# Farama-Foundation/Miniworld

Hardware: AMD Instinct MI355X
Metric: env-steps/s (batched, 80x60 RGB) (higher is better)
Workload: dtype f32

## Files before the change

include/mwengine.h:

```cpp
#ifndef MWENGINE_H
#define MWENGINE_H
#include <stdint.h>
#ifdef __cplusplus
extern "C" {
#endif

#define MW_ABI_VERSION 4

enum {
    MW_OK = 0,
    MW_E_INVALID = -1,
    MW_E_HIP = -2,
    MW_E_NOMEM = -3,
    MW_E_CAPACITY = -4,
    MW_E_DEVICE = -5,
    MW_E_OVERFLOW = -6
};

enum { MW_ENT_NONE = 0, MW_ENT_BOX = 1, MW_ENT_MESH = 2, MW_ENT_FRAME = 3 };

enum {
    MW_TASK_NONE = 0,
    MW_TASK_GOTO = 1,
    MW_TASK_PICKUP = 2,
// ... 246 lines not shown
int mw_debug_set_nav_passes(mw_engine *e, int32_t *d_passes);

int mw_check(mw_engine *e, void *stream);

int mw_kernel_time_ms(mw_engine *e, int32_t reset, double *raster_ms, double *setup_ms, int64_t *launches);

int mw_get_info(mw_engine *e, int32_t *d_health, double *d_ent_pos, int32_t ent_slot, void *stream);
int mw_get_final_info(mw_engine *e, int32_t *d_health, double *d_goal_pos, void *stream);
int mw_get_reset_pending(mw_engine *e, uint8_t *d_out, void *stream);

int mw_set_frame_reuse(mw_engine *e, int32_t on);
int mw_get_frame_clean(mw_engine *e, uint8_t *d_out, void *stream);

int mw_set_frame_cache(mw_engine *e, int32_t slots);
int mw_get_frame_source(mw_engine *e, uint8_t *d_out, void *stream);

int mw_get_list_lengths(mw_engine *e, int32_t first_env, int32_t count, int32_t *host_out, void *stream);

int mw_debug_set_mesh_frame_seq(mw_engine *e, uint32_t seq);
int mw_debug_get_slow_heads(mw_engine *e, uint32_t *host_out, void *stream);

enum { MW_PATH_TILE = 0, MW_PATH_QUAD = 1, MW_PATH_QUAD_MESH = 2, MW_PATH_GENERIC = 3 };
int mw_raster_path(const mw_engine *e);

#ifdef __cplusplus
}
#endif
#endif
```

miniworld_amd/csrc/mw_engine.h:

```cpp
#pragma once
#include <hip/hip_runtime.h>

#include <algorithm>
#include <cstdarg>
#include <cstdio>
#include <cstdlib>
#include <memory>
#include <string>
#include <utility>
#include <vector>

#include "mw_assets.h"
#include "mw_device.h"
#include "mw_kernels.h"
#include "mw_policy.h"

#define MW_TIMING_STRIDE 8

template <typename H, hipError_t (*destroy)(H)>
struct Destroy { void operator()(H h) const { (void)destroy(h); } };
template <typename T>
using DevBuf = std::unique_ptr<T, Destroy<void *, hipFree>>;
using Stream = std::unique_ptr<ihipStream_t, Destroy<hipStream_t, hipStreamDestroy>>;
using Event = std::unique_ptr<ihipEvent_t, Destroy<hipEvent_t, hipEventDestroy>>;
// ... 79 lines not shown
    bool frame_reuse = false;
    struct { uint8_t *obs = nullptr; float *depth = nullptr; int layout = 0; bool valid = false; } held;
    struct {
        int slots = 0;
        DevBuf<uint8_t> frames;
        DevBuf<float> depth;
        DevBuf<uint64_t> meta;
        DevBuf<MwFcArgs> d_args;
        MwFcArgs args{};
        bool args_stale = true;
        bool with_depth = false;
        bool dirty = true;
    } fc;
    uint32_t *d_plan[2] = {nullptr, nullptr};
    int plan_cur = 0;
    struct {
        int depth = 0, pad = 0, layout = 0, cur = 0;
        uint8_t *ring = nullptr, *final_stack = nullptr;
        size_t frame_bytes = 0;
        int64_t pushes = 0;
        uint8_t *flags = nullptr;
    } stack;
    MwSnapConfig snap_cfg{};
    MwSnapLayout snap_layout{};
    MwSnapTable *d_snap_tab = nullptr;
    int snap_chunks_per_item = 0;
    Event ev_refill_done;
};

namespace mwhost {
// ... 124 lines not shown
```

miniworld_amd/csrc/mw_engine.hip:

```cpp
#include <cmath>
#include <cstring>

#include "mw_engine.h"
#include "mw_rng.h"

namespace mwhost {
thread_local std::string g_create_error;
}
using namespace mwhost;

namespace {

void seed_env(const mw_engine *e, uint64_t *rng, int i, uint64_t seed)
{
    const size_t N = (size_t)e->cfg.num_envs;
    uint64_t w[5];
    mw::rng_seed_words(e->cfg.rng_mode == MW_RNG_PCG64, seed, w);
    for (int k = 0; k < 5; ++k) rng[(size_t)k * N + i] = w[k];
}

int upload_textures(mw_engine *e)
{
    const size_t table = (size_t)MW_MAX_TEX * sizeof(MwTexDesc) / 4;
    size_t total = table;
// ... 159 lines not shown
    ALLOC(a.rec_cull, (size_t)N * a.max_vis * MW_CULL_REC);
    if (has_visiting_order(cfg->max_visible)) {
        ALLOC(a.rec_order, (size_t)N * (a.max_vis + 1));
    }
    if (cfg->max_polys > 64 && !(getenv("MW_OCC_CACHE") && atoi(getenv("MW_OCC_CACHE")) == 0)) {
        ALLOC(a.occ_valid, e->n_sets);
        ALLOC(a.occ_cache, (size_t)e->n_sets * MW_OCC_CACHE_STRIDE(cfg->max_polys));
    }
    { const auto pick = [](int id) { return id >= MW_SC_pending_remove; }; MW_WORLD_FIELDS(LIVE_ALLOC) }
    ALLOC(a.frame_clean, (size_t)N);
    ALLOC(a.fc_key, (size_t)MW_FC_KEY_WORDS * N); ALLOC(a.fc_epoch, (size_t)N); ALLOC(a.fc_source, (size_t)N);
    HIP_TRY(e, hipMemset(a.pending_remove, 0xFF, 4 * (size_t)N));
    ALLOC(a.nvis, N); ALLOC(a.envhdr, (size_t)MW_ENVHDR * N); ALLOC(a.status, 1);
    ALLOC(e->d_reward_scratch, N); ALLOC(e->d_flag_scratch, 2 * (size_t)N);
    ALLOC(e->d_final_list, 1 + (size_t)N);
    ALLOC(e->d_plan[0], MW_PLAN_WORDS(N)); ALLOC(e->d_plan[1], MW_PLAN_WORDS(N));
    ALLOC(e->stack.flags, 2 * (size_t)N);
    ALLOC(e->d_mask, N); ALLOC(e->d_step_override, 3 * (size_t)N);
#ifdef MW_PERF_HOOKS
    if (getenv("MW_K1_PROF")) ALLOC(a.k1_prof, MW_K1_PROF_SLOTS * (size_t)N);
    if (getenv("MW_ENT_PROF")) ALLOC(e->d_ent_prof, (size_t)16 * 2 * N * MW_MAX_MESH_ENTS * 8);
    if (getenv("MW_K2Q_PROF")) ALLOC(e->d_k2q_prof, (size_t)N * 96);
#endif
#undef LIVE_ALLOC
#undef ALLOC
    {
        std::vector<int32_t> m1((size_t)N, -1);
        HIP_TRY(e, hipMemcpy(a.carry, m1.data(), 4 * (size_t)N, hipMemcpyHostToDevice));
        std::vector<uint64_t> seeds(5 * (size_t)N, 0);
        for (int i = 0; i < N; ++i) seed_env(e, seeds.data(), i, (uint64_t)i);
        HIP_TRY(e, hipMemcpy(a.rng, seeds.data(), 40 * (size_t)N, hipMemcpyHostToDevice));
// ... 516 lines not shown
    if (!d_health && !d_goal_pos) return fail(e, MW_E_INVALID, "mw_get_final_info: nothing asked for");
    if (d_health && !e->args.final_health) return fail(e, MW_E_INVALID, "mw_get_final_info: this engine's task keeps no health (MW_TASK_COLLECT only)");
    return launch_info(e, 1, e->args.final_health, e->args.final_goal, 0, d_health, d_goal_pos, stream);
}

int mw_get_reset_pending(mw_engine *e, uint8_t *d_out, void *stream)
{
    return e ? get_env_bytes(e, "mw_get_reset_pending", e->args.reset_pending, d_out, stream) : MW_E_INVALID;
}

int mw_get_frame_source(mw_engine *e, uint8_t *d_out, void *stream)
{
    return e ? get_env_bytes(e, "mw_get_frame_source", e->args.fc_source, d_out, stream) : MW_E_INVALID;
}

int mw_get_frame_clean(mw_engine *e, uint8_t *d_out, void *stream)
{
    return e ? get_env_bytes(e, "mw_get_frame_clean", e->args.frame_clean, d_out, stream) : MW_E_INVALID;
}

int mw_kernel_time_ms(mw_engine *e, int32_t reset, double *raster_ms, double *setup_ms, int64_t *launches)
{
    if (!e) return MW_E_INVALID;
    ON_DEVICE(e);
    double r = 0, s = 0;
    int64_t n = 0;
    for (auto &ev : e->ev_used) {
        (void)hipEventSynchronize(ev.c.get());
        float t1 = 0, t2 = 0;
        (void)hipEventElapsedTime(&t1, ev.a.get(), ev.b.get());
// ... 20 lines not shown
```

miniworld_amd/csrc/mw_engine_frame.hip:

```cpp
#include "mw_engine.h"

using namespace mwhost;

namespace {

template <typename K>
K k1_of(const mw_engine *e, int lanes, K wave, K wave_pcg, K dense, K dense_pcg)
{
    const bool pcg = e->cfg.rng_mode == MW_RNG_PCG64;
    if (lanes) return pcg ? dense_pcg : dense;
    return pcg ? wave_pcg : wave;
}
#define MW_K1(e, lanes, stem) k1_of(e, lanes, stem##_kernel, stem##_pcg_kernel, stem##_dense_kernel, stem##_dense_pcg_kernel)

template <typename... A>
struct KernelPair {
    void (*plain)(A...);
    void (*sub)(A..., const int32_t *);
};
template <typename... A>
KernelPair<A...> kernel_pair(void (*plain)(A...), void (*sub)(A..., const int32_t *)) { return {plain, sub}; }
#define MW_PAIR(stem) kernel_pair(stem##_kernel, stem##_sub_kernel)

template <typename... A, typename... P>
// ... 205 lines not shown
void launch_quad(const mw_engine *e, const Frame &f, int part, hipStream_t st, const uint32_t *plan = nullptr)
{
    const MwArgs &a = f.a;
    const int lds = mw_rasterq_lds_bytes(e->cfg.msaa, a.W, a.H, a.n_tiles, f.depth ? 1 : 0);
    launch(f.p.quad4 ? MW_PAIR(mw_rasterq4) : MW_PAIR(mw_rasterq), f.list, dim3(e->cfg.num_envs), dim3(MWQ_THREADS), (size_t)lds, st, a.N, a.W, a.H, a.max_vis,
           a.tiles_x, a.n_tiles, (const float *)a.rec_raster, (const float *)a.rec_shade, (const float *)a.rec_cull,
           (const int32_t *)a.nvis, (const float *)a.envhdr, a.texels, f.obs, f.depth, raster_flags(e->dbg_flags, e->obs_layout, part, 0u, false), e->texel_bytes, e->d_k2q_prof,
           plan && f.pol.cache ? (const MwFcArgs *)e->fc.d_args.get() : nullptr, plan);
}

const uint32_t *launch_plan(mw_engine *e, const Frame &f, hipStream_t st)
{
    const MwArgs &a = f.a; const int N = e->cfg.num_envs;
    uint32_t *plan = e->d_plan[e->plan_cur], *next = e->d_plan[e->plan_cur ^ 1];
    e->plan_cur ^= 1;
    hipLaunchKernelGGL(mw_frame_plan_kernel, dim3((N + MW_PLAN_ENVS - 1) / MW_PLAN_ENVS), dim3(64), 0, st, N, f.pol.reuse ? 1 : 0, (const uint8_t *)a.frame_clean,
                       (const uint64_t *)a.fc_key, f.pol.cache ? (const uint64_t *)e->fc.meta.get() : nullptr, f.pol.cache ? e->fc.slots : 0, a.fc_source, plan, next);
    return plan;
}

void launch_tiles(const mw_engine *e, const Frame &f, int part, hipStream_t st)
{
    const MwArgs &a = f.a; const mw_engine::MeshPath &m = e->mp;
    const TileLaunch t = tile_launch(part, a.tile_list != nullptr, f.p.big, a.max_vis, a.n_tiles, e->waves_per_env, e->cfg.num_envs, m.mesh_tile_waves);
    launch(tile_kernel_of(f.p.big, f.p.depth, f.p.general, f.p.ragged, f.p.mesh, t.part == 1), f.list, dim3(t.grid), dim3(64), t.lds, st,
           a.N, a.W, a.H, a.max_vis, a.tiles_x, a.n_tiles, t.waves_per_env, t.tiles_per_wave, (const float *)a.rec_raster, (const float *)a.rec_shade,
           (const float *)a.rec_cull, (const int32_t *)a.nvis, (const float *)a.envhdr, a.tex, a.texels, f.obs, f.depth, raster_flags(e->dbg_flags, e->obs_layout, t.part, f.mf.stamp, f.pol.reuse),
           e->texel_bytes, (const uint16_t *)a.rec_order, a.mesh_pos, a.mesh_nrm, a.mesh_rgb, a.mesh_uv, m.keys.get(),
           (const float *)m.plane_cache.get(), m.plane_cap, (const float4 *)m.slow_frags.get(), (const uint32_t *)m.slow_head.get(),
           (const uint32_t *)a.tile_list, a.ent_list_n, a.tile_list_cap, std::max(a.n_xcc, 1), (const uint8_t *)a.frame_clean);
}

// ... 366 lines not shown
```

miniworld_amd/csrc/mw_engine_kernels.hip:

```cpp
#include "mw_kernels.h"

extern "C" __global__ void mw_info_kernel(int N, int E, const int32_t *health, const double *epos, int slot, int32_t *out_health, double *out_pos)
{
    const int i = blockIdx.x * blockDim.x + threadIdx.x;
    if (i >= N) return;
    if (out_health) out_health[i] = health[i];
    if (out_pos)
        for (int c = 0; c < 3; ++c) out_pos[(size_t)i * 3 + c] = epos[((size_t)c * E + slot) * N + i];
}

extern "C" __global__ __launch_bounds__(1024) void mw_final_list_kernel(int N, const uint8_t *__restrict__ pending, int32_t *__restrict__ pending_remove,
                                                                       int32_t *__restrict__ list)
{
    __shared__ int s_wave[16];
    const int tid = (int)threadIdx.x, lane = tid & 63, wave = tid >> 6;
    int base = 0;
    for (int i0 = 0; i0 < N; i0 += 1024) {
        const int i = i0 + tid;
        const bool p = i < N && pending[i] != 0;
        const unsigned long long m = __ballot(p);
        if (lane == 0) s_wave[wave] = __popcll(m);
        __syncthreads();
        int before = base, total = 0;
        for (int w = 0; w < 16; ++w) {
// ... 18 lines not shown
    if ((int)blockIdx.x >= list[0]) return;
    const size_t env = (size_t)list[1 + blockIdx.x];
    const uint8_t *src = obs + env * row_bytes;
    uint8_t *dst = final_obs + env * row_bytes;
    if ((((uintptr_t)obs | (uintptr_t)final_obs | (uintptr_t)row_bytes) & 15u) == 0) {
        for (size_t k = threadIdx.x; k < row_bytes / 16; k += blockDim.x)
            reinterpret_cast<uint4 *>(dst)[k] = reinterpret_cast<const uint4 *>(src)[k];
    } else {
        for (size_t k = threadIdx.x; k < row_bytes; k += blockDim.x) dst[k] = src[k];
    }
    if (depth && final_depth)
        for (int k = threadIdx.x; k < depth_row; k += blockDim.x) final_depth[env * depth_row + k] = depth[env * depth_row + k];
}

extern "C" __global__ __launch_bounds__(64) void mw_frame_plan_kernel(int N, int reuse, const uint8_t *__restrict__ frame_clean, const uint64_t *__restrict__ key,
                                                                     const uint64_t *__restrict__ meta, int slots, uint8_t *__restrict__ frame_source,
                                                                     uint32_t *__restrict__ plan, uint32_t *__restrict__ next)
{
    const int lane = (int)threadIdx.x, env = (int)blockIdx.x * MW_PLAN_ENVS + lane;
    if (blockIdx.x == 0 && lane < 2) next[lane] = 0u;
    const bool on = env < N;
    uint32_t v = MW_SRC_CLEAN;
    if (on) {
        const bool clean = frame_clean[env] != 0;
        uint32_t match = 0u, header = 0u;
        if (meta) {
            const uint64_t *row = static_cast<const uint64_t *>(__builtin_assume_aligned(meta + (size_t)env * MW_FC_META_WORDS(slots), 16));
            const uint64_t *cur = static_cast<const uint64_t *>(__builtin_assume_aligned(key + (size_t)env * MW_FC_KEY_WORDS, 16));
            header = (uint32_t)row[0];
#pragma unroll
            for (int j = 0; j < MW_FC_MAX_SLOTS; ++j) {
                const int jj = j < slots ? j : slots - 1;
                match |= mw_fc_key_equal(static_cast<const uint64_t *>(__builtin_assume_aligned(row + 2 + MW_FC_KEY_WORDS * jj, 16)), cur) && j < slots ? 1u << j : 0u;
            }
        }
        v = mw_frame_verdict(clean, reuse != 0, match, header, meta ? slots : 0);
        frame_source[env] = (uint8_t)v;
    }
    const uint32_t src = v & 0xFFu;
    const bool draw = on && src == MW_SRC_DRAWN, copy = on && src >= (uint32_t)MW_SRC_SLOT(0);
    const uint64_t md = __builtin_amdgcn_ballot_w64(draw), mc = __builtin_amdgcn_ballot_w64(copy), below = (1ull << lane) - 1ull;
    unsigned long long base = 0ull;
    if (lane == 0 && (md | mc))
        base = atomicAdd(reinterpret_cast<unsigned long long *>(plan), (unsigned long long)__popcll(md) | (unsigned long long)__popcll(mc) << 32);
    const uint32_t bd = (uint32_t)__builtin_amdgcn_readfirstlane((int)(uint32_t)base), bc = (uint32_t)__builtin_amdgcn_readfirstlane((int)(uint32_t)(base >> 32));
    const uint32_t entry = (uint32_t)env | (v >> 8) << MW_PLAN_ENV_BITS;
    const uint32_t id = bd + (uint32_t)__popcll(md & below), ic = bc + (uint32_t)__popcll(mc & below);
    if (draw && id < (uint32_t)N) plan[MW_PLAN_HEAD + id] = entry;
    if (copy && ic < (uint32_t)N) plan[MW_PLAN_HEAD + (size_t)N + ic] = entry;
}
```

miniworld_amd/csrc/mw_frame_plan.h:

```cpp
#pragma once
#include <stdint.h>

#include "mw_hd.h"

#ifndef MW_FC_KEY_WORDS
#define MW_FC_KEY_WORDS 10
#define MW_FC_META_WORDS(slots) (2 + MW_FC_KEY_WORDS * (slots))
#define MW_FC_MAX_SLOTS 8
#endif

#define MW_SRC_DRAWN 0
#define MW_SRC_CLEAN 1
#define MW_SRC_SLOT(j) (2 + (j))

#define MW_PLAN_HEAD 4
#define MW_PLAN_WORDS(N) (MW_PLAN_HEAD + 2 * (size_t)(N))
#define MW_PLAN_ENV_BITS 24
#define MW_PLAN_ENV_MASK 0xFFFFFFu

MW_HD uint32_t mw_frame_verdict(bool clean, bool reuse, uint32_t match, uint32_t header, int slots)
{
    if (reuse && clean) return MW_SRC_CLEAN;
    if (slots <= 0) return MW_SRC_DRAWN;
    match &= (1u << slots) - 1u;
    if (match) {
        uint32_t hit = 0;
        while (!((match >> hit) & 1u)) ++hit;
        return (uint32_t)MW_SRC_SLOT(hit) | hit << 8;
    }
    const uint32_t last = (uint32_t)(slots - 1);
    return MW_SRC_DRAWN | (header < last ? header : last) << 8;
}

// ... 15 lines not shown
```

miniworld_amd/csrc/mw_kernels.h:

```cpp
#pragma once
#include "mw_device.h"
#include "mw_frame_plan.h"
#include "mw_snapshot.h"
#include "mw_snapframes.h"
#include "mw_state_view.h"
#include "mw_nav.h"

#define MW_KERNEL_PAIR(stem, ...)                          \
    extern "C" __global__ void stem##_kernel(__VA_ARGS__); \
    extern "C" __global__ void stem##_sub_kernel(__VA_ARGS__, const int32_t *list)

#define MW_K1_ARGS MwArgs a, int lanes_per_env, const int32_t *__restrict__ actions, float *__restrict__ reward, \
                   uint8_t *__restrict__ term, uint8_t *__restrict__ trunc
extern "C" __global__ void mw_step_setup_kernel(MW_K1_ARGS);
extern "C" __global__ void mw_step_setup_pcg_kernel(MW_K1_ARGS);
extern "C" __global__ void mw_step_setup_dense_kernel(MW_K1_ARGS);
extern "C" __global__ void mw_step_setup_dense_pcg_kernel(MW_K1_ARGS);
#define MW_K1_REPEAT_ARGS MW_K1_ARGS, int repeat, int32_t *__restrict__ nsteps
extern "C" __global__ void mw_step_repeat_kernel(MW_K1_REPEAT_ARGS);
extern "C" __global__ void mw_step_repeat_pcg_kernel(MW_K1_REPEAT_ARGS);
extern "C" __global__ void mw_step_repeat_dense_kernel(MW_K1_REPEAT_ARGS);
extern "C" __global__ void mw_step_repeat_dense_pcg_kernel(MW_K1_REPEAT_ARGS);
#define MW_K1_PLAN_ARGS MW_K1_ARGS, int horizon, int32_t *__restrict__ nsteps, float *__restrict__ step_reward, int frameless
extern "C" __global__ void mw_step_plan_kernel(MW_K1_PLAN_ARGS);
// ... 108 lines not shown

#define MW_SNAPF_ARGS MwSnapfArgs a, uint32_t *__restrict__ status
extern "C" __global__ void mw_snapshot_save_frames_kernel(MW_SNAPF_ARGS, const uint8_t *__restrict__ obs, const uint8_t *__restrict__ depth,
                                                          const uint8_t *__restrict__ ring, const uint8_t *__restrict__ stack_flags,
                                                          uint8_t *__restrict__ frames, MW_SNAP_ITEMS);
extern "C" __global__ void mw_snapshot_load_frames_kernel(MW_SNAPF_ARGS, const uint8_t *__restrict__ frames, uint8_t *__restrict__ obs,
                                                          uint8_t *__restrict__ depth, uint8_t *__restrict__ ring, uint8_t *__restrict__ stack_flags,
                                                          MW_SNAP_ITEMS);

extern "C" __global__ void mw_info_kernel(int N, int E, const int32_t *health, const double *epos, int slot, int32_t *out_health, double *out_pos);
extern "C" __global__ void mw_final_list_kernel(int N, const uint8_t *__restrict__ pending, int32_t *__restrict__ pending_remove, int32_t *__restrict__ list);
extern "C" __global__ void mw_final_copy_kernel(const int32_t *__restrict__ list, const uint8_t *__restrict__ obs, uint8_t *__restrict__ final_obs,
                                                unsigned long long row_bytes, const float *__restrict__ depth, float *__restrict__ final_depth, int depth_row);
#define MW_PLAN_ENVS 64
extern "C" __global__ void mw_frame_plan_kernel(int N, int reuse, const uint8_t *__restrict__ frame_clean, const uint64_t *__restrict__ key,
                                                const uint64_t *__restrict__ meta, int slots, uint8_t *__restrict__ frame_source,
                                                uint32_t *__restrict__ plan, uint32_t *__restrict__ next);

#define MW_SV_THREADS 256
#define MW_SV_ENVS (MW_SV_THREADS / 64)
extern "C" __global__ void mw_state_get_kernel(MwStateArrays a, mw_state_view v, int N, int E, int first_env, int count);
extern "C" __global__ void mw_state_set_where_kernel(MwStateArrays a, mw_state_view v, const uint8_t *__restrict__ mask, int N, int E,
                                                     uint32_t *__restrict__ status, uint8_t *__restrict__ reset_pending,
                                                     uint8_t *__restrict__ frame_clean, uint32_t *__restrict__ fc_epoch,
                                                     uint8_t *__restrict__ stack_flags);

#define MW_NAV_THREADS 512
#define MW_NAV_QUERY_THREADS 256
extern "C" __global__ void mw_nav_build_kernel(MwNavArgs a, mw_nav_params p, const uint8_t *__restrict__ mask, const double *__restrict__ d_target,
                                               uint16_t *__restrict__ field, int32_t *__restrict__ passes);
extern "C" __global__ void mw_nav_query_kernel(MwNavArgs a, mw_nav_params p, const double *__restrict__ d_target, const uint16_t *__restrict__ field,
                                               const double *__restrict__ pos, int32_t *__restrict__ cost, int32_t *__restrict__ next,
// ... 5 lines not shown
```

miniworld_amd/csrc/mw_policy.h:

```cpp
#pragma once
#include <stddef.h>
#include <stdint.h>

#include "../../include/mwengine.h"
#include "mw_shape.h"
#include "mw_snapframes.h"
#include "mw_snapshot.h"

namespace mwpolicy {

inline bool tile_kernels_exact(int W, int H) { return W <= 128 && H <= 128 && W * H <= 128 * 96; }

inline int tiles_across(int W) { return (W + MW_TILE_W - 1) / MW_TILE_W; }
inline int tiles_down(int H) { return (H + MW_TILE_H - 1) / MW_TILE_H; }
inline bool frame_on_grid(int W, int H) { return W % MW_TILE_W == 0 && H % MW_TILE_H == 0; }
inline bool tile_path_ok(int W, int H) { return frame_on_grid(W, H) && tile_kernels_exact(W, H); }
inline bool frame_size_ok(int W, int H) { return W >= 1 && H >= 1 && W <= 255 * MW_TILE_W && H <= 255 * MW_TILE_H; }

inline bool has_visiting_order(int max_visible) { return max_visible > 64; }

inline int geom_lanes(int max_polys, int max_ents, bool order)
{
    const int items = 2 * (max_polys + 6 * max_ents + 1);
    int L = 8;
// ... 101 lines not shown
};
inline FramePolicy frame_policy(const FrameFacts &f)
{
    const bool plain = (f.kind == CALL_RENDER || f.kind == CALL_STEP) && f.view_flags == 0;
    const bool seeded_pass = f.seeded && (f.kind == CALL_TERMINAL_STEP || f.kind == CALL_LIST_PASS) && f.view_flags == 0;
    const bool plain_step = (plain && f.kind == CALL_STEP) || (seeded_pass && f.kind == CALL_TERMINAL_STEP), bare = !f.meshes && f.dbg_flags == 0;
    const bool source = plain_step && f.path == MW_PATH_QUAD;
    return {f.frame_reuse && plain_step && bare && f.held_match, source,
            source && f.cache_allocated && bare && f.layout == MW_OBS_HWC_U8 && f.task != MW_TASK_COLLECT, plain || seeded_pass};
}

inline bool frame_plans(const FramePolicy &pol, int path, bool listed, int N)
{
    return !listed && path == MW_PATH_QUAD && (pol.reuse || pol.cache) && N <= 0xFFFFFF;
}

struct TileLaunch { int part, waves_per_env, tiles_per_wave, grid; size_t lds; };
inline TileLaunch tile_launch(int part, bool tile_list, bool big, int max_vis, int n_tiles, int wpe, int N, int mesh_tile_waves)
{
    const int lds_recs = max_vis < MW_LDS_RECS ? max_vis : MW_LDS_RECS;
    const size_t lds = big ? 192 : (size_t)lds_recs * (MW_LDS_SHADE_Q + MW_LDS_CULL_Q) * 16 + 192;
    const bool listed = part == 2 && tile_list;
    if (listed) part = 3;
    const int wpe2 = part == 2 ? n_tiles : wpe, tpw2 = part == 2 ? 1 : (n_tiles + wpe - 1) / wpe;
    const int all = N * n_tiles;
    return {part, wpe2, tpw2, listed ? (mesh_tile_waves < all ? mesh_tile_waves : all) : (N + 7) / 8 * 8 * wpe2, lds};
}

inline bool wide_units(uintptr_t bits) { return (bits & 15u) == 0; }

// ... 41 lines not shown
```

miniworld_amd/csrc/mw_rasterq.hip:

```cpp
#include "mw_mesh.h"
#include "mw_kernels.h"

#define MWQ_WAVES (MWQ_THREADS / 64)
#define MWQ_CAP_MAX 48
#define MWQ_SLOTS 16
#define MWQ_EMPTY 63u
#ifndef MWQ_TILE_FALLBACK
#define MWQ_TILE_FALLBACK 1
#endif
#ifndef MWQ_OCC
#define MWQ_OCC 6
#endif

namespace {

__device__ inline bool wave_all(bool p) { return __builtin_amdgcn_ballot_w64(p) == __builtin_amdgcn_read_exec(); }
__device__ inline bool wave_any(bool p) { return __builtin_amdgcn_ballot_w64(p) != 0ull; }

enum { QC_FALLBACK = 0, QC_BIG, QC_EXACT, QC_P4, QC_P3, QC_P2, QC_P1, QC_TRIV, QC_SKY, QC_NCLS, QC_NONE = 15 };

template <int S> struct QRec {
    static constexpr int TQ = (S + 3) / 4;
    static constexpr int SH = 4 + 3 * TQ;
    static constexpr int CT = SH + 6;
// ... 439 lines not shown
        wins &= valid;
        if (!wave_any(wins)) continue;
        const float4 *rec = recp(valid ? p : 0);
        const RGB c = shade_lane(rec + QRec<S>::SH, cx.te, fx + 0.5f, fy + 0.5f);
#pragma unroll
        for (int s = 0; s < S; ++s) {
            const bool eq = valid && pid[s] == (uint32_t)p;
            q.r[s] = eq ? c.r : q.r[s]; q.g[s] = eq ? c.g : q.g[s]; q.b[s] = eq ? c.b : q.b[s];
        }
    }
    store_pixel<S>(cx, q, key[0] >> 16, px, py, on);
}

#ifdef MW_PERF_HOOKS
#define MWQ_WG_BEGIN() const unsigned long long wg_t0 = prof ? __builtin_amdgcn_s_memrealtime() : 0ull
#define MWQ_WG_END(kind) do { if (prof && (threadIdx.x & 63) == 0) { unsigned long long *w_ = prof + (size_t)N * (MWQ_WAVES * 8 + 16) + (size_t)blockIdx.x * 16; \
    if (threadIdx.x == 0) { w_[0] = wg_t0; w_[1] = (kind); } w_[2 + (threadIdx.x >> 6)] = __builtin_amdgcn_s_memrealtime(); } } while (0)
#else
#define MWQ_WG_BEGIN() do {} while (0)
#define MWQ_WG_END(kind) do {} while (0)
#endif
template <int S, bool SUB = false>
__device__ inline void rasterq_body(
    int N, int W, int H, int max_vis, int tiles_x, int n_tiles,
    const float *__restrict__ rec_raster, const float *__restrict__ rec_shade, const float *__restrict__ rec_cull,
    const int32_t *__restrict__ nvis_arr, const float *__restrict__ envhdr, const uint32_t *__restrict__ texels,
    uint8_t *__restrict__ obs, float *__restrict__ depth, int dbg, int texel_bytes, unsigned long long *__restrict__ prof,
    const MwFcArgs *__restrict__ fc, const uint32_t *__restrict__ plan, const int32_t *__restrict__ list = nullptr)
{
    extern __shared__ __attribute__((aligned(16))) unsigned char smem[];
    typedef QRec<S> R;
    MWQ_WG_BEGIN();
    int env = blockIdx.x;
    const int tid = threadIdx.x, lane = tid & 63, wave = tid >> 6;
    const bool has_depth = depth != nullptr;
    uint32_t fc_victim = 0u;
    if (SUB) {
        if (env >= list[0]) return;
        env = list[1 + env];
    } else if (env >= N) return;
    else if (plan) {
        const uint32_t b = blockIdx.x, n_draw = plan[0];
        if (b < n_draw) {
            const uint32_t entry = plan[MW_PLAN_HEAD + b];
            env = (int)(entry & MW_PLAN_ENV_MASK);
            fc_victim = entry >> MW_PLAN_ENV_BITS;
        } else {
            if (b - n_draw >= plan[1] || !fc) { MWQ_WG_END(3); return; }
            const uint32_t entry = plan[MW_PLAN_HEAD + (size_t)N + (b - n_draw)];
            env = (int)(entry & MW_PLAN_ENV_MASK);
            const int hit = (int)(entry >> MW_PLAN_ENV_BITS), fc_slots = fc->slots;
            const int fbytes = W * H * 3;
            const uint8_t *src = fc->frames + ((size_t)env * fc_slots + hit) * fbytes;
            uint8_t *dst = obs + (size_t)env * fbytes;
            if ((reinterpret_cast<uintptr_t>(dst) & 15u) == 0u)
                for (int i = tid; i < fbytes / 16; i += MWQ_THREADS) reinterpret_cast<uint4 *>(dst)[i] = reinterpret_cast<const uint4 *>(src)[i];
            else if ((reinterpret_cast<uintptr_t>(dst) & 3u) == 0u)
                for (int i = tid; i < fbytes / 4; i += MWQ_THREADS) reinterpret_cast<uint32_t *>(dst)[i] = reinterpret_cast<const uint32_t *>(src)[i];
            else
                for (int i = tid; i < fbytes; i += MWQ_THREADS) dst[i] = src[i];
            if (has_depth) {
                const float *zs = fc->depth + ((size_t)env * fc_slots + hit) * (W * H);
                float *zd = depth + (size_t)env * (W * H);
                if ((reinterpret_cast<uintptr_t>(zd) & 15u) == 0u)
                    for (int i = tid; i < W * H / 4; i += MWQ_THREADS) reinterpret_cast<float4 *>(zd)[i] = reinterpret_cast<const float4 *>(zs)[i];
                else
                    for (int i = tid; i < W * H; i += MWQ_THREADS) zd[i] = zs[i];
            }
            MWQ_WG_END(2);
            return;
        }
    }
    const QPlan pl = q_plan(S, W, H, n_tiles, has_depth);
    float4 *s_rec = reinterpret_cast<float4 *>(smem + pl.rec);
    uint8_t *s_frame = smem + pl.frame;
    uint16_t *s_z = reinterpret_cast<uint16_t *>(smem + pl.zbuf);
    uint32_t *s_qids = reinterpret_cast<uint32_t *>(smem + pl.qids);
    uint16_t *s_queue = reinterpret_cast<uint16_t *>(smem + pl.queue);
    uint16_t *s_xq = reinterpret_cast<uint16_t *>(smem + pl.xq);
    uint32_t *s_tcnt = reinterpret_cast<uint32_t *>(smem + pl.tcnt);
    uint32_t *s_tfull = reinterpret_cast<uint32_t *>(smem + pl.tfull);
    uint8_t *s_tlist = smem + pl.tlist;
    uint32_t *s_tmask = reinterpret_cast<uint32_t *>(smem + pl.tmask);
    uint32_t *s_pe = reinterpret_cast<uint32_t *>(smem + pl.pe);
// ... 231 lines not shown
            const int Q = Q0 + tid;
            const uint32_t cls = Q < nquads ? s_qids[Q] >> 24 : (uint32_t)QC_NONE;
            const uint32_t base = (uint32_t)__builtin_amdgcn_ds_bpermute((int)(cls & 15u) << 2, (int)fb_lane);
            if (cls != QC_NONE) s_queue[base * 16u + s_rank[Q]] = (uint16_t)Q;
        }
        for (uint32_t b = tid; b < first_bat[QC_NCLS]; b += MWQ_THREADS) {
            uint32_t cls = 0u;
#pragma unroll
            for (int c = 1; c < QC_NCLS; ++c) cls += b >= first_bat[c] ? 1u : 0u;
            uint32_t cfirst = 0u, cslot = 0u, ccnt = 0u;
#pragma unroll
            for (int c = 0; c < QC_NCLS; ++c) { cfirst = cls == (uint32_t)c ? first_bat[c] : cfirst; cslot = cls == (uint32_t)c ? first_b[c] : cslot; ccnt = cls == (uint32_t)c ? cnt_c[c] : ccnt; }
            const uint32_t size = cls == QC_TRIV ? 64u : 16u, bi = b - cfirst;
            s_btab[b] = ((cslot + bi * (size / 16u)) * 16u) | (cls << 12) | (min(size, ccnt - bi * size) << 16);
        }
        __syncthreads();

        stamp(4);
        if (prof && tid < QC_NCLS) prof[(size_t)N * MWQ_WAVES * 8 + (size_t)env * 16 + tid] = s_misc[tid];
        const uint32_t sky_u8 = sky_bytes<S>(cx);
        const uint32_t n_batches = (dbg & 0x400) ? 0u : first_bat[QC_NCLS];
        for (;;) {
            uint32_t b = 0u;
            if (lane == 0) b = atomicAdd(&s_misc[17], 1u);
            b = (uint32_t)__builtin_amdgcn_readfirstlane((int)b);
            if (b >= n_batches) break;
            const uint32_t be = (uint32_t)__builtin_amdgcn_readfirstlane((int)s_btab[b]);
            const int cls = (int)((be >> 12) & 15u);
            if ((dbg & 0x800) && cls != QC_TRIV) continue;
            if ((dbg & 0x1000) && cls == QC_TRIV) continue;
// ... 110 lines not shown
    if (!SUB && fc) {
        const int fc_slots = fc->slots;
        const uint32_t victim = s_misc[20];
        uint64_t *meta = fc->meta + (size_t)env * MW_FC_META_WORDS(fc_slots);
        uint4 *fd = reinterpret_cast<uint4 *>(fc->frames + ((size_t)env * fc_slots + victim) * (npix * 3));
        const uint4 *src = reinterpret_cast<const uint4 *>(s_frame);
        for (int i = tid; i < npix * 3 / 16; i += MWQ_THREADS) fd[i] = src[i];
        if (has_depth) {
            float *fz = fc->depth + ((size_t)env * fc_slots + victim) * npix;
            for (int i = tid; i < npix; i += MWQ_THREADS) fz[i] = depth_of(i);
        }
        if (tid < MW_FC_KEY_WORDS / 2)
            reinterpret_cast<uint4 *>(meta + 2 + MW_FC_KEY_WORDS * victim)[tid] = reinterpret_cast<const uint4 *>(fc->key + (size_t)env * MW_FC_KEY_WORDS)[tid];
        if (tid == 64) meta[0] = (uint64_t)(victim + 1u == (uint32_t)fc_slots ? 0u : victim + 1u);
    }
    MWQ_WG_END(0);
}

}

#define MWQ_FWD N, W, H, max_vis, tiles_x, n_tiles, rec_raster, rec_shade, rec_cull, nvis_arr, envhdr, texels, obs, depth, dbg, texel_bytes, prof, fc, plan
#define MWQ_PAIR(stem, bounds, ...)                                                                          \
    extern "C" __global__ bounds void stem##_kernel(MWQ_ARGS) { rasterq_body<__VA_ARGS__, false>(MWQ_FWD); } \
    extern "C" __global__ bounds void stem##_sub_kernel(MWQ_ARGS, const int32_t *__restrict__ list) { rasterq_body<__VA_ARGS__, true>(MWQ_FWD, list); }
MWQ_PAIR(mw_rasterq, __launch_bounds__(MWQ_THREADS, MWQ_OCC), 8)
MWQ_PAIR(mw_rasterq4, __launch_bounds__(MWQ_THREADS), 4)

extern "C" int mw_rasterq_lds_bytes(int S, int W, int H, int n_tiles, int depth) { return q_plan(S, W, H, n_tiles, depth != 0).total; }
extern "C" int mw_rasterq_cap(int depth) { return q_cap(depth != 0); }

#ifdef MWQ_PROBE
// ... 16 lines not shown
```

miniworld_amd/engine.py:

```python
from __future__ import annotations

import ctypes as C
import os
import subprocess

import numpy as np

_CSRC = os.path.join(os.path.dirname(os.path.abspath(__file__)), "csrc")
LIB_PATH = os.environ.get("MW_ENGINE_LIB") or os.path.join(_CSRC, "libmwengine.so")

ABI_VERSION = 4
MAX_REPEAT = 256
MAX_PLAN = MAX_REPEAT
MAX_STACK = 16
STACK_PAD_RESET, STACK_PAD_ZERO = 0, 1
SNAPF_DEPTH, SNAPF_STACK = 1, 2
ENT_NONE, ENT_BOX, ENT_MESH, ENT_FRAME = 0, 1, 2, 3
POLY_ENTITY = 0x100
POLY_XF = 0x200
POLY_QUAD = 0x400
TASK_NONE, TASK_GOTO, TASK_PICKUP, TASK_PUTNEXT, TASK_SIDEWALK, TASK_SIGN, TASK_COLLECT = 0, 1, 2, 3, 4, 5, 6
GEN_NONE, GEN_HALLWAY, GEN_ONEROOM, GEN_PICKUP, GEN_MAZE, GEN_PROGRAM = 0, 1, 2, 3, 4, 5
OP_COIN, OP_DRAW_DIR, OP_PLACE, OP_FIXED, OP_BOX_SIZE, OP_COLOR, OP_APPEND = 1, 2, 3, 4, 5, 6, 7
PROG_MAX_ROOMS, PROG_MAX_TEX, PROG_MAX_OPS, PROG_MAX_ENTS = 16, 8, 48, 64
AUTORESET_OFF, AUTORESET_SAME_STEP, AUTORESET_NEXT_STEP = 0, 1, 2
OBS_HWC_U8, OBS_CWH_U8, OBS_GREY_F64 = 0, 1, 2
RNG_PHILOX, RNG_PCG64 = 0, 1
PATH_TILE, PATH_QUAD, PATH_QUAD_MESH, PATH_GENERIC = 0, 1, 2, 3

EXPORTS = [
    "mw_create", "mw_destroy", "mw_last_error", "mw_upload_texture", "mw_upload_mesh",
    "mw_set_geometry", "mw_get_geometry", "mw_set_state", "mw_get_state", "mw_set_step_params", "mw_reset",
    "mw_step", "mw_step_repeat", "mw_step_plan", "mw_step_plan_trace", "mw_render", "mw_render_top", "mw_render_view", "mw_visible_ents", "mw_set_obs_layout", "mw_pcg64_draws", "mw_check", "mw_kernel_time_ms", "mw_raster_path", "mw_get_info", "mw_get_final_info", "mw_get_reset_pending", "mw_set_frame_reuse", "mw_get_frame_clean", "mw_set_frame_cache", "mw_get_frame_source", "mw_set_final_obs", "mw_get_list_lengths", "mw_debug_set_mesh_frame_seq", "mw_debug_get_slow_heads",
    "mw_set_gen_program", "mw_selftest_rcp", "mw_selftest_div", "mw_selftest_sort", "mw_selftest_q",
    "mw_selftest_sincosf",
    "mw_set_frame_stack", "mw_stack_refresh", "mw_stack_window",
    "mw_snapshot_bytes", "mw_snapshot_save", "mw_snapshot_load",
    "mw_snapshot_frames_bytes", "mw_snapshot_save_frames", "mw_snapshot_load_frames",
    "mw_snapshot_save_at", "mw_snapshot_save_frames_at", "mw_snapshot_load_where", "mw_snapshot_load_frames_where",
    "mw_reset_where", "mw_set_reset_seeds",
    "mw_get_state_device", "mw_set_state_where",
    "mw_nav_build", "mw_nav_query", "mw_debug_set_nav_passes",
]


class MwRange(C.Structure):
    _fields_ = [("default", C.c_double), ("lo", C.c_double), ("hi", C.c_double)]

# ... 179 lines not shown
    L.mw_snapshot_save_at.argtypes = [vp, vp, vp, i32, vp, i32, vp]
    L.mw_snapshot_save_frames_at.argtypes = [vp, vp, vp, i32, vp, vp, vp, i32, i32, vp]
    L.mw_snapshot_load_where.argtypes = [vp, vp, vp, vp, i32, i32, vp]
    L.mw_snapshot_load_frames_where.argtypes = [vp, vp, vp, vp, i32, i32, i32, vp, vp, vp]
    L.mw_pcg64_draws.argtypes = [C.c_uint64, i32, vp, vp]
    L.mw_check.argtypes = [vp, vp]
    L.mw_kernel_time_ms.argtypes = [vp, i32, C.POINTER(C.c_double), C.POINTER(C.c_double), C.POINTER(C.c_int64)]
    L.mw_raster_path.argtypes = [vp]
    L.mw_get_info.argtypes = [vp, vp, vp, i32, vp]
    L.mw_get_final_info.argtypes = [vp, vp, vp, vp]
    L.mw_get_reset_pending.argtypes = [vp, vp, vp]
    L.mw_set_frame_reuse.argtypes = [vp, i32]
    L.mw_get_frame_clean.argtypes = [vp, vp, vp]
    L.mw_set_frame_cache.argtypes = [vp, i32]
    L.mw_get_frame_source.argtypes = [vp, vp, vp]
    L.mw_get_list_lengths.argtypes = [vp, i32, i32, vp, vp]
    L.mw_debug_set_mesh_frame_seq.argtypes = [vp, C.c_uint32]
    L.mw_debug_get_slow_heads.argtypes = [vp, vp, vp]
    _lib = L
    return L


def frame_reuse_allowed() -> bool:
    return os.environ.get("MW_FRAME_REUSE", "1").strip() != "0"


MAX_FRAME_CACHE = 8


def frame_cache_allowed() -> bool:
# ... 515 lines not shown
    def set_frame_reuse(self, on: bool):
        on = bool(on) and frame_reuse_allowed()
        self._check(self.lib.mw_set_frame_reuse(self.h, int(on)), "mw_set_frame_reuse")
        self.frame_reuse = on
        return on

    def set_frame_cache(self, slots: int):
        slots = int(slots) if frame_cache_allowed() else 0
        self._check(self.lib.mw_set_frame_cache(self.h, slots), "mw_set_frame_cache")
        self.frame_cache = slots
        return slots

    def get_frame_source(self, out=None):
        return self._get_bytes("mw_get_frame_source", out)

    def get_frame_clean(self, out=None):
        return self._get_bytes("mw_get_frame_clean", out)

    def list_lengths(self):
        out = np.zeros(self.N, np.int32)
        self._check(self.lib.mw_get_list_lengths(self.h, 0, self.N, out.ctypes.data, _stream_ptr(self.device)), "mw_get_list_lengths")
        return out

    def raster_path(self):
        return int(self.lib.mw_raster_path(self.h))

    def kernel_time_ms(self, reset=0):
        r, s, n = C.c_double(), C.c_double(), C.c_int64()
        self._check(self.lib.mw_kernel_time_ms(self.h, reset, C.byref(r), C.byref(s), C.byref(n)), "mw_kernel_time_ms")
        return r.value, s.value, n.value
# ... 31 lines not shown
```

Measured before the change: 17.04 million.

## Order drawn frames by visible-list cost class so heavy envs launch first

The frame plan kernel now buckets drawn environments into eight cost classes by their visible-primitive count and counts them with per-class packed atomics. The quad raster kernel maps block indices to classes from heaviest to lightest, so expensive environments start first and the tail imbalance shrinks. It costs extra ballots and atomics in the plan kernel, a larger plan buffer, and some index arithmetic per raster block. A host-side plan readback API and extra profiling fields are added as well.

```diff
diff --git a/include/mwengine.h b/include/mwengine.h
--- a/include/mwengine.h
+++ b/include/mwengine.h
@@ -284,6 +284,7 @@
 
 int mw_set_frame_cache(mw_engine *e, int32_t slots);
 int mw_get_frame_source(mw_engine *e, uint8_t *d_out, void *stream);
+int mw_get_frame_plan(mw_engine *e, uint32_t *host_plan, int64_t words, int32_t *host_lengths, void *stream);
 
 int mw_get_list_lengths(mw_engine *e, int32_t first_env, int32_t count, int32_t *host_out, void *stream);
 
diff --git a/miniworld_amd/csrc/mw_engine.h b/miniworld_amd/csrc/mw_engine.h
--- a/miniworld_amd/csrc/mw_engine.h
+++ b/miniworld_amd/csrc/mw_engine.h
@@ -117,6 +117,7 @@
     } fc;
     uint32_t *d_plan[2] = {nullptr, nullptr};
     int plan_cur = 0;
+    bool plan_made = false;
     struct {
         int depth = 0, pad = 0, layout = 0, cur = 0;
         uint8_t *ring = nullptr, *final_stack = nullptr;
diff --git a/miniworld_amd/csrc/mw_engine.hip b/miniworld_amd/csrc/mw_engine.hip
--- a/miniworld_amd/csrc/mw_engine.hip
+++ b/miniworld_amd/csrc/mw_engine.hip
@@ -197,7 +197,7 @@
     ALLOC(a.nvis, N); ALLOC(a.envhdr, (size_t)MW_ENVHDR * N); ALLOC(a.status, 1);
     ALLOC(e->d_reward_scratch, N); ALLOC(e->d_flag_scratch, 2 * (size_t)N);
     ALLOC(e->d_final_list, 1 + (size_t)N);
-    ALLOC(e->d_plan[0], MW_PLAN_WORDS(N)); ALLOC(e->d_plan[1], MW_PLAN_WORDS(N));
+    ALLOC(e->d_plan[0], MW_PLAN_WORDS(N, frame_plan_ordered(N))); ALLOC(e->d_plan[1], MW_PLAN_WORDS(N, frame_plan_ordered(N)));
     ALLOC(e->stack.flags, 2 * (size_t)N);
     ALLOC(e->d_mask, N); ALLOC(e->d_step_override, 3 * (size_t)N);
 #ifdef MW_PERF_HOOKS
@@ -744,6 +744,20 @@
     return e ? get_env_bytes(e, "mw_get_frame_source", e->args.fc_source, d_out, stream) : MW_E_INVALID;
 }
 
+int mw_get_frame_plan(mw_engine *e, uint32_t *host_plan, int64_t words, int32_t *host_lengths, void *stream)
+{
+    if (!e || !host_plan || !host_lengths) return fail(e, MW_E_INVALID, "mw_get_frame_plan: null argument");
+    const int N = e->cfg.num_envs;
+    const size_t want = MW_PLAN_WORDS(N, frame_plan_ordered(N));
+    if (words != (int64_t)want) return fail(e, MW_E_INVALID, "mw_get_frame_plan: %lld words given, the block has %zu", (long long)words, want);
+    if (!e->plan_made) return fail(e, MW_E_INVALID, "mw_get_frame_plan: no frame of this engine has been planned yet");
+    ON_DEVICE(e);
+    HIP_TRY(e, hipStreamSynchronize((hipStream_t)stream));
+    HIP_TRY(e, hipMemcpy(host_plan, e->d_plan[e->plan_cur ^ 1], want * sizeof(uint32_t), hipMemcpyDeviceToHost));
+    HIP_TRY(e, hipMemcpy(host_lengths, e->args.nvis, sizeof(int32_t) * (size_t)N, hipMemcpyDeviceToHost));
+    return MW_OK;
+}
+
 int mw_get_frame_clean(mw_engine *e, uint8_t *d_out, void *stream)
 {
     return e ? get_env_bytes(e, "mw_get_frame_clean", e->args.frame_clean, d_out, stream) : MW_E_INVALID;
diff --git a/miniworld_amd/csrc/mw_engine_frame.hip b/miniworld_amd/csrc/mw_engine_frame.hip
--- a/miniworld_amd/csrc/mw_engine_frame.hip
+++ b/miniworld_amd/csrc/mw_engine_frame.hip
@@ -243,8 +243,10 @@
     const MwArgs &a = f.a; const int N = e->cfg.num_envs;
     uint32_t *plan = e->d_plan[e->plan_cur], *next = e->d_plan[e->plan_cur ^ 1];
     e->plan_cur ^= 1;
+    e->plan_made = true;
     hipLaunchKernelGGL(mw_frame_plan_kernel, dim3((N + MW_PLAN_ENVS - 1) / MW_PLAN_ENVS), dim3(64), 0, st, N, f.pol.reuse ? 1 : 0, (const uint8_t *)a.frame_clean,
-                       (const uint64_t *)a.fc_key, f.pol.cache ? (const uint64_t *)e->fc.meta.get() : nullptr, f.pol.cache ? e->fc.slots : 0, a.fc_source, plan, next);
+                       (const uint64_t *)a.fc_key, f.pol.cache ? (const uint64_t *)e->fc.meta.get() : nullptr, f.pol.cache ? e->fc.slots : 0,
+                       frame_plan_ordered(N) ? (const int32_t *)a.nvis : nullptr, a.fc_source, plan, next);
     return plan;
 }
 
diff --git a/miniworld_amd/csrc/mw_engine_kernels.hip b/miniworld_amd/csrc/mw_engine_kernels.hip
--- a/miniworld_amd/csrc/mw_engine_kernels.hip
+++ b/miniworld_amd/csrc/mw_engine_kernels.hip
@@ -56,15 +56,23 @@
 }
 
 extern "C" __global__ __launch_bounds__(64) void mw_frame_plan_kernel(int N, int reuse, const uint8_t *__restrict__ frame_clean, const uint64_t *__restrict__ key,
-                                                                     const uint64_t *__restrict__ meta, int slots, uint8_t *__restrict__ frame_source,
-                                                                     uint32_t *__restrict__ plan, uint32_t *__restrict__ next)
+                                                                     const uint64_t *__restrict__ meta, int slots, const int32_t *__restrict__ nvis,
+                                                                     uint8_t *__restrict__ frame_source, uint32_t *__restrict__ plan, uint32_t *__restrict__ next)
 {
     const int lane = (int)threadIdx.x, env = (int)blockIdx.x * MW_PLAN_ENVS + lane;
-    if (blockIdx.x == 0 && lane < 2) next[lane] = 0u;
+    const bool ordered = nvis != nullptr;
+    if (blockIdx.x == 0) {
+        if (lane < 2) next[lane] = 0u;
+        else if (lane < 4) next[MW_PLAN_CLS_LO + lane - 2] = 0u;
+        else if (lane < 6) next[MW_PLAN_CLS_HI + lane - 4] = 0u;
+        else if (lane == 6) plan[2] = ordered ? (uint32_t)MW_PLAN_CLASSES : 0u;
+    }
     const bool on = env < N;
     uint32_t v = MW_SRC_CLEAN;
+    uint32_t cls = 0u;
     if (on) {
         const bool clean = frame_clean[env] != 0;
+        const int32_t len = ordered ? nvis[env] : 0;
         uint32_t match = 0u, header = 0u;
         if (meta) {
             const uint64_t *row = static_cast<const uint64_t *>(__builtin_assume_aligned(meta + (size_t)env * MW_FC_META_WORDS(slots), 16));
@@ -78,16 +86,33 @@
         }
         v = mw_frame_verdict(clean, reuse != 0, match, header, meta ? slots : 0);
         frame_source[env] = (uint8_t)v;
+        cls = mw_plan_cost_class(len);
     }
     const uint32_t src = v & 0xFFu;
     const bool draw = on && src == MW_SRC_DRAWN, copy = on && src >= (uint32_t)MW_SRC_SLOT(0);
     const uint64_t md = __builtin_amdgcn_ballot_w64(draw), mc = __builtin_amdgcn_ballot_w64(copy), below = (1ull << lane) - 1ull;
-    unsigned long long base = 0ull;
-    if (lane == 0 && (md | mc))
-        base = atomicAdd(reinterpret_cast<unsigned long long *>(plan), (unsigned long long)__popcll(md) | (unsigned long long)__popcll(mc) << 32);
-    const uint32_t bd = (uint32_t)__builtin_amdgcn_readfirstlane((int)(uint32_t)base), bc = (uint32_t)__builtin_amdgcn_readfirstlane((int)(uint32_t)(base >> 32));
+    unsigned long long add = (unsigned long long)__popcll(md) | (unsigned long long)__popcll(mc) << 32, add_lo = 0ull, add_hi = 0ull;
+    uint64_t mine = md;
+    if (ordered) {
+#pragma unroll
+        for (uint32_t c = 0; c < MW_PLAN_CLASSES; ++c) {
+            const uint64_t m = __builtin_amdgcn_ballot_w64(draw && cls == c);
+            (c < 4u ? add_lo : add_hi) |= (unsigned long long)__popcll(m) << (16u * (c & 3u));
+            mine = cls == c ? m : mine;
+        }
+    }
+    unsigned long long old = 0ull;
+    if (lane < 3) {
+        const unsigned long long a = lane == 0 ? add : lane == 1 ? add_lo : add_hi;
+        uint32_t *at = plan + (lane == 0 ? 0 : lane == 1 ? MW_PLAN_CLS_LO : MW_PLAN_CLS_HI);
+        if (a) old = atomicAdd(reinterpret_cast<unsigned long long *>(at), a);
+    }
+    const uint32_t old_lo = (uint32_t)old, old_hi = (uint32_t)(old >> 32);
+    const uint32_t bd = (uint32_t)__builtin_amdgcn_readlane((int)old_lo, 0), bc = (uint32_t)__builtin_amdgcn_readlane((int)old_hi, 0);
+    const uint64_t base_lo = (uint64_t)(uint32_t)__builtin_amdgcn_readlane((int)old_lo, 1) | (uint64_t)(uint32_t)__builtin_amdgcn_readlane((int)old_hi, 1) << 32;
+    const uint64_t base_hi = (uint64_t)(uint32_t)__builtin_amdgcn_readlane((int)old_lo, 2) | (uint64_t)(uint32_t)__builtin_amdgcn_readlane((int)old_hi, 2) << 32;
     const uint32_t entry = (uint32_t)env | (v >> 8) << MW_PLAN_ENV_BITS;
-    const uint32_t id = bd + (uint32_t)__popcll(md & below), ic = bc + (uint32_t)__popcll(mc & below);
-    if (draw && id < (uint32_t)N) plan[MW_PLAN_HEAD + id] = entry;
-    if (copy && ic < (uint32_t)N) plan[MW_PLAN_HEAD + (size_t)N + ic] = entry;
+    const uint32_t id = (ordered ? mw_plan_class_count(base_lo, base_hi, cls) : bd) + (uint32_t)__popcll(mine & below), ic = bc + (uint32_t)__popcll(mc & below);
+    if (draw && id < (uint32_t)N) plan[MW_PLAN_DRAW(N, ordered ? cls : 0u) + id] = entry;
+    if (copy && ic < (uint32_t)N) plan[MW_PLAN_COPY(N) + ic] = entry;
 }
diff --git a/miniworld_amd/csrc/mw_frame_plan.h b/miniworld_amd/csrc/mw_frame_plan.h
--- a/miniworld_amd/csrc/mw_frame_plan.h
+++ b/miniworld_amd/csrc/mw_frame_plan.h
@@ -13,10 +13,39 @@
 #define MW_SRC_CLEAN 1
 #define MW_SRC_SLOT(j) (2 + (j))
 
-#define MW_PLAN_HEAD 4
-#define MW_PLAN_WORDS(N) (MW_PLAN_HEAD + 2 * (size_t)(N))
+#define MW_PLAN_HEAD 96
+#define MW_PLAN_CLS_LO 32
+#define MW_PLAN_CLS_HI 64
+#define MW_PLAN_CLASSES 8
+#define MW_PLAN_COPY(N) ((size_t)MW_PLAN_HEAD)
+#define MW_PLAN_DRAW(N, c) (MW_PLAN_HEAD + (size_t)(N) * (1u + (size_t)(c)))
+#define MW_PLAN_WORDS(N, ordered) (MW_PLAN_HEAD + (size_t)(N) * ((ordered) ? 1u + MW_PLAN_CLASSES : 2u))
 #define MW_PLAN_ENV_BITS 24
 #define MW_PLAN_ENV_MASK 0xFFFFFFu
+#define MW_PLAN_ORDERED_MAX_N 0xFFFF
+
+MW_HD uint32_t mw_plan_cost_class(int32_t nvis)
+{
+    if (nvis <= 0) return 0u;
+    const uint32_t c = (uint32_t)nvis >> 2;
+    return c < MW_PLAN_CLASSES - 1u ? c : MW_PLAN_CLASSES - 1u;
+}
+
+MW_HD uint32_t mw_plan_class_count(uint64_t lo, uint64_t hi, uint32_t c)
+{
+    return (uint32_t)((c < 4u ? lo : hi) >> (16u * (c & 3u))) & 0xFFFFu;
+}
+
+MW_HD bool mw_plan_slot(uint32_t b, const uint32_t *count, uint32_t *cls, uint32_t *rank)
+{
+    uint32_t first = 0u;
+    for (int c = MW_PLAN_CLASSES - 1; c >= 0; --c) {
+        if (b - first < count[c]) { *cls = (uint32_t)c; *rank = b - first; return true; }
+        first += count[c];
+    }
+    *cls = 0u; *rank = b - first;
+    return false;
+}
 
 MW_HD uint32_t mw_frame_verdict(bool clean, bool reuse, uint32_t match, uint32_t header, int slots)
 {
diff --git a/miniworld_amd/csrc/mw_kernels.h b/miniworld_amd/csrc/mw_kernels.h
--- a/miniworld_amd/csrc/mw_kernels.h
+++ b/miniworld_amd/csrc/mw_kernels.h
@@ -146,8 +146,8 @@
                                                 unsigned long long row_bytes, const float *__restrict__ depth, float *__restrict__ final_depth, int depth_row);
 #define MW_PLAN_ENVS 64
 extern "C" __global__ void mw_frame_plan_kernel(int N, int reuse, const uint8_t *__restrict__ frame_clean, const uint64_t *__restrict__ key,
-                                                const uint64_t *__restrict__ meta, int slots, uint8_t *__restrict__ frame_source,
-                                                uint32_t *__restrict__ plan, uint32_t *__restrict__ next);
+                                                const uint64_t *__restrict__ meta, int slots, const int32_t *__restrict__ nvis,
+                                                uint8_t *__restrict__ frame_source, uint32_t *__restrict__ plan, uint32_t *__restrict__ next);
 
 #define MW_SV_THREADS 256
 #define MW_SV_ENVS (MW_SV_THREADS / 64)
diff --git a/miniworld_amd/csrc/mw_policy.h b/miniworld_amd/csrc/mw_policy.h
--- a/miniworld_amd/csrc/mw_policy.h
+++ b/miniworld_amd/csrc/mw_policy.h
@@ -139,6 +139,10 @@
 {
     return !listed && path == MW_PATH_QUAD && (pol.reuse || pol.cache) && N <= 0xFFFFFF;
 }
+inline bool frame_plan_ordered(int N)
+{
+    return N <= 0xFFFF;
+}
 
 struct TileLaunch { int part, waves_per_env, tiles_per_wave, grid; size_t lds; };
 inline TileLaunch tile_launch(int part, bool tile_list, bool big, int max_vis, int n_tiles, int wpe, int N, int mesh_tile_waves)
diff --git a/miniworld_amd/csrc/mw_rasterq.hip b/miniworld_amd/csrc/mw_rasterq.hip
--- a/miniworld_amd/csrc/mw_rasterq.hip
+++ b/miniworld_amd/csrc/mw_rasterq.hip
@@ -477,11 +477,11 @@
 
 #ifdef MW_PERF_HOOKS
 #define MWQ_WG_BEGIN() const unsigned long long wg_t0 = prof ? __builtin_amdgcn_s_memrealtime() : 0ull
-#define MWQ_WG_END(kind) do { if (prof && (threadIdx.x & 63) == 0) { unsigned long long *w_ = prof + (size_t)N * (MWQ_WAVES * 8 + 16) + (size_t)blockIdx.x * 16; \
-    if (threadIdx.x == 0) { w_[0] = wg_t0; w_[1] = (kind); } w_[2 + (threadIdx.x >> 6)] = __builtin_amdgcn_s_memrealtime(); } } while (0)
+#define MWQ_WG_END(kind, env_, nvis_) do { if (prof && (threadIdx.x & 63) == 0) { unsigned long long *w_ = prof + (size_t)N * (MWQ_WAVES * 8 + 16) + (size_t)blockIdx.x * 16; \
+    if (threadIdx.x == 0) { w_[0] = wg_t0; w_[1] = (kind); w_[10] = (unsigned long long)(env_); w_[11] = (unsigned long long)(nvis_); } w_[2 + (threadIdx.x >> 6)] = __builtin_amdgcn_s_memrealtime(); } } while (0)
 #else
 #define MWQ_WG_BEGIN() do {} while (0)
-#define MWQ_WG_END(kind) do {} while (0)
+#define MWQ_WG_END(kind, env_, nvis_) do {} while (0)
 #endif
 template <int S, bool SUB = false>
 __device__ inline void rasterq_body(
@@ -503,14 +503,25 @@
         env = list[1 + env];
     } else if (env >= N) return;
     else if (plan) {
-        const uint32_t b = blockIdx.x, n_draw = plan[0];
-        if (b < n_draw) {
-            const uint32_t entry = plan[MW_PLAN_HEAD + b];
+        const uint32_t b = blockIdx.x, n_copy = plan[1], n_classes = plan[2];
+        const uint64_t c_lo = *reinterpret_cast<const uint64_t *>(plan + MW_PLAN_CLS_LO), c_hi = *reinterpret_cast<const uint64_t *>(plan + MW_PLAN_CLS_HI);
+        uint32_t n_draw = plan[0], cls = 0u, rank = b;
+        bool draws = b < n_draw;
+        if (n_classes != 0u) {
+            uint32_t count[MW_PLAN_CLASSES];
+#pragma unroll
+            for (uint32_t c = 0; c < MW_PLAN_CLASSES; ++c) count[c] = mw_plan_class_count(c_lo, c_hi, c);
+            draws = mw_plan_slot(b, count, &cls, &rank);
+            n_draw = b - rank;
+        }
+        if (draws) {
+            if (rank >= (uint32_t)N) { MWQ_WG_END(3, 0, 0); return; }
+            const uint32_t entry = plan[MW_PLAN_DRAW(N, cls) + rank];
             env = (int)(entry & MW_PLAN_ENV_MASK);
             fc_victim = entry >> MW_PLAN_ENV_BITS;
         } else {
-            if (b - n_draw >= plan[1] || !fc) { MWQ_WG_END(3); return; }
-            const uint32_t entry = plan[MW_PLAN_HEAD + (size_t)N + (b - n_draw)];
+            if (b - n_draw >= n_copy || !fc) { MWQ_WG_END(3, 0, 0); return; }
+            const uint32_t entry = plan[MW_PLAN_COPY(N) + (b - n_draw)];
             env = (int)(entry & MW_PLAN_ENV_MASK);
             const int hit = (int)(entry >> MW_PLAN_ENV_BITS), fc_slots = fc->slots;
             const int fbytes = W * H * 3;
@@ -530,7 +541,7 @@
                 else
                     for (int i = tid; i < W * H; i += MWQ_THREADS) zd[i] = zs[i];
             }
-            MWQ_WG_END(2);
+            MWQ_WG_END(2, env, 0);
             return;
         }
     }
@@ -792,6 +803,14 @@
             const uint32_t size = cls == QC_TRIV ? 64u : 16u, bi = b - cfirst;
             s_btab[b] = ((cslot + bi * (size / 16u)) * 16u) | (cls << 12) | (min(size, ccnt - bi * size) << 16);
         }
+#ifdef MW_PERF_HOOKS
+        if (prof && tid == 0) {
+            unsigned long long *c_ = prof + (size_t)N * MWQ_WAVES * 8 + (size_t)env * 16, pk[3] = {0ull, 0ull, 0ull};
+            for (int c = 0; c < QC_NCLS; ++c) pk[c >> 2] |= (c_[c] < 0xFFFFull ? c_[c] : 0xFFFFull) << (16 * (c & 3));
+            pk[2] |= (c_[12] < 0xFFFFull ? c_[12] : 0xFFFFull) << 16;
+            c_[9] = pk[0]; c_[10] = pk[1]; c_[11] = pk[2]; c_[12] = s_misc[16];
+        }
+#endif
         __syncthreads();
 
         stamp(4);
@@ -932,7 +951,7 @@
             reinterpret_cast<uint4 *>(meta + 2 + MW_FC_KEY_WORDS * victim)[tid] = reinterpret_cast<const uint4 *>(fc->key + (size_t)env * MW_FC_KEY_WORDS)[tid];
         if (tid == 64) meta[0] = (uint64_t)(victim + 1u == (uint32_t)fc_slots ? 0u : victim + 1u);
     }
-    MWQ_WG_END(0);
+    MWQ_WG_END(0, env, nvis);
 }
 
 }
diff --git a/miniworld_amd/engine.py b/miniworld_amd/engine.py
--- a/miniworld_amd/engine.py
+++ b/miniworld_amd/engine.py
@@ -31,7 +31,7 @@
 EXPORTS = [
     "mw_create", "mw_destroy", "mw_last_error", "mw_upload_texture", "mw_upload_mesh",
     "mw_set_geometry", "mw_get_geometry", "mw_set_state", "mw_get_state", "mw_set_step_params", "mw_reset",
-    "mw_step", "mw_step_repeat", "mw_step_plan", "mw_step_plan_trace", "mw_render", "mw_render_top", "mw_render_view", "mw_visible_ents", "mw_set_obs_layout", "mw_pcg64_draws", "mw_check", "mw_kernel_time_ms", "mw_raster_path", "mw_get_info", "mw_get_final_info", "mw_get_reset_pending", "mw_set_frame_reuse", "mw_get_frame_clean", "mw_set_frame_cache", "mw_get_frame_source", "mw_set_final_obs", "mw_get_list_lengths", "mw_debug_set_mesh_frame_seq", "mw_debug_get_slow_heads",
+    "mw_step", "mw_step_repeat", "mw_step_plan", "mw_step_plan_trace", "mw_render", "mw_render_top", "mw_render_view", "mw_visible_ents", "mw_set_obs_layout", "mw_pcg64_draws", "mw_check", "mw_kernel_time_ms", "mw_raster_path", "mw_get_info", "mw_get_final_info", "mw_get_reset_pending", "mw_set_frame_reuse", "mw_get_frame_clean", "mw_set_frame_cache", "mw_get_frame_source", "mw_get_frame_plan", "mw_set_final_obs", "mw_get_list_lengths", "mw_debug_set_mesh_frame_seq", "mw_debug_get_slow_heads",
     "mw_set_gen_program", "mw_selftest_rcp", "mw_selftest_div", "mw_selftest_sort", "mw_selftest_q",
     "mw_selftest_sincosf",
     "mw_set_frame_stack", "mw_stack_refresh", "mw_stack_window",
@@ -241,6 +241,7 @@
     L.mw_get_frame_clean.argtypes = [vp, vp, vp]
     L.mw_set_frame_cache.argtypes = [vp, i32]
     L.mw_get_frame_source.argtypes = [vp, vp, vp]
+    L.mw_get_frame_plan.argtypes = [vp, vp, C.c_int64, vp, vp]
     L.mw_get_list_lengths.argtypes = [vp, i32, i32, vp, vp]
     L.mw_debug_set_mesh_frame_seq.argtypes = [vp, C.c_uint32]
     L.mw_debug_get_slow_heads.argtypes = [vp, vp, vp]
@@ -786,6 +787,22 @@
     def get_frame_source(self, out=None):
         return self._get_bytes("mw_get_frame_source", out)
 
+    def get_frame_plan(self):
+        N = self.N
+        ordered = N <= 0xFFFF
+        block = np.zeros(96 + N * (9 if ordered else 2), np.uint32)
+        lengths = np.zeros(N, np.int32)
+        self._check(self.lib.mw_get_frame_plan(self.h, block.ctypes.data, block.size, lengths.ctypes.data, _stream_ptr(self.device)), "mw_get_frame_plan")
+        n_draw, n_copy, classes = int(block[0]), int(block[1]), int(block[2])
+        packed = [int(block[32]) | int(block[33]) << 32, int(block[64]) | int(block[65]) << 32]
+        counts = [(packed[c >> 2] >> (16 * (c & 3))) & 0xFFFF for c in range(8)] if classes else []
+        if classes:
+            draw = np.concatenate([block[96 + N * (1 + c):96 + N * (1 + c) + min(counts[c], N)] for c in reversed(range(8))])
+        else:
+            draw = block[96 + N:96 + N + min(n_draw, N)].copy()
+        return {"n_draw": n_draw, "n_copy": n_copy, "classes": classes, "class_counts": counts, "draw": draw,
+                "copy": block[96:96 + min(n_copy, N)].copy(), "lengths": lengths, "block": block}
+
     def get_frame_clean(self, out=None):
         return self._get_bytes("mw_get_frame_clean", out)
 
```

Result: faster. 17.70 million, median of 6 (+3.9%).
